# google-research/corenet

Measured on AMD Instinct MI355X. Metric: voxels/sec fwd+bwd @128^3, higher is better.
Workload: dtype bf16x3 (the convolutions of decoder stages 3-6 and the encoder's 3x3 convolutions -- forward of stages 4-5, data gradient of all -- multiply operands split into two bf16 terms: three bf16 MFMAs per product, fp32 accumulation, 16 mantissa bits, ~3e-6 relative per layer; tensors, everything else and t

## Files before the change

corenet_amd/_lib.py:

```python
from __future__ import annotations

import ctypes as C
import os
from typing import Optional

import torch as t

_HERE = os.path.dirname(os.path.abspath(__file__))
TOOLS_LIB_PATH = os.path.join(os.path.dirname(_HERE), "tools", "_build", "libcorenet_hip_tools.so")
PROBE_LIB_PATH = os.path.join(os.path.dirname(_HERE), "tools", "_build", "libcrn_probe.so")
LIB_PATH = os.environ.get("CORENET_HIP_LIB", TOOLS_LIB_PATH if os.environ.get("CRN_TOOLS_LIB") == "1" else
                          os.path.join(_HERE, "lib", "libcorenet_hip.so"))

c_i32p = C.POINTER(C.c_int32)
c_f32p = C.c_void_p
vp = C.c_void_p
i64 = C.c_int64
i32 = C.c_int
f32 = C.c_float
sz = C.c_size_t


class CrnTapBoxes(C.Structure):
  _fields_ = [("n_groups", C.c_int32), ("c_groups", C.c_int32), ("n_box", (C.c_int8 * 6) * 8),
# ... 19 lines not shown
  pass


_SIGS = {
    "crn_conv_fwd": [C.POINTER(CrnView), C.POINTER(CrnInTransform), vp, i32, vp, i32,
                     C.POINTER(CrnView), i32, i32, i32, i32, i32, i32, i32, i32, vp, vp],
    "crn_conv_fwd_bf3": [C.POINTER(CrnView), C.POINTER(CrnInTransform), vp, i32, vp, i32,
                         C.POINTER(CrnView), i32, i32, i32, i32, i32, i32, i32, vp, vp],
    "crn_conv_fwd_bf3_slabs": [C.POINTER(CrnView), C.POINTER(CrnInTransform), vp, i32, vp, i32,
                               C.POINTER(CrnView), i32, i32, i32, i32, i32, i32, i32, vp, vp],
    "crn_conv_fwd_bf3_slabs_bnbwd": [C.POINTER(CrnView), C.POINTER(CrnInTransform), vp, i32, vp, i32,
                                     C.POINTER(CrnView), i32, i32, i32, i32, i32, i32, i32, vp, C.POINTER(CrnBnBwdFuse), vp],
    "crn_conv_fwd_bf3_slabs_stats": [C.POINTER(CrnView), C.POINTER(CrnInTransform), vp, i32, vp, i32,
                                     C.POINTER(CrnView), i32, i32, i32, i32, i32, i32, i32, vp, i32, vp, sz, C.POINTER(C.c_int), vp],
    "crn_batch_renorm_bwd_apply": [vp, i64, vp, i64, i32, i32, i64, i32, vp, vp, vp, vp, vp, i64, vp, vp, i32, vp, i32,
                                   vp, sz, i32, vp],
    "crn_conv_wgrad_bf3": [C.POINTER(CrnView), C.POINTER(CrnInTransform), C.POINTER(CrnView), vp, i32,
                           i32, i32, i32, i32, i32, i32, i32, vp],
    "crn_conv_wgrad_bf3_boxes": [C.POINTER(CrnView), C.POINTER(CrnInTransform), C.POINTER(CrnView), vp, i32,
                                 i32, i32, i32, i32, i32, i32, i32, vp, vp],
    "crn_conv_wgrad": [C.POINTER(CrnView), C.POINTER(CrnInTransform), C.POINTER(CrnView), vp, i32,
                       i32, i32, i32, i32, i32, i32, i32, vp, vp],
    "crn_bf3_operands": [vp, vp, i32, i64, vp, vp],
    "crn_bf3_gather_image": [vp, vp, i32, vp, vp],
    "crn_convt_s2k7_fwd_bf3": [vp, i64, i32, i32, i32, i32, C.POINTER(CrnInTransform), vp, vp, vp, i64, i64, i32, vp],
    "crn_convt_s2k7_dgrad_bf3": [vp, i64, i64, i32, i32, i32, i32, i32, vp, vp, i64, i32, vp],
    "crn_convt_s2k7_c2_fwd_bf3": [vp, i64, i32, i32, i32, i32, C.POINTER(CrnInTransform), vp, vp, vp, i64, i64, i32, vp],
    "crn_convt_s2k7_c2_dgrad_bf3": [vp, i64, i64, i32, i32, i32, i32, i32, vp, vp, i64, i32, vp],
    "crn_convt_s2k7_wgrad_bf3": [vp, i64, i32, i32, i32, i32, C.POINTER(CrnInTransform), vp, i64, i64, i32, vp, i32, i32, vp, vp],
    "crn_convt_s2k7_ximage": [vp, i64, i32, i32, i32, i32, C.POINTER(CrnInTransform), vp, sz, vp],
    "crn_splitk_defer": [i32],
    "crn_splitk_reserve": [i64, vp],
    "crn_splitk_release": [vp],
    "crn_set_deterministic": [i32],
    "crn_roctx_push": [C.c_char_p],
    "crn_roctx_pop": [],
    "crn_comm_unique_id": [vp],
    "crn_comm_init": [vp, i32, i32, C.POINTER(vp)],
    "crn_comm_destroy": [vp],
    "crn_comm_info": [vp, C.POINTER(i32), C.POINTER(i32), C.POINTER(i32)],
    "crn_allreduce_f32": [vp, vp, i64, vp],
    "crn_broadcast_f32": [vp, vp, i64, i32, vp],
    "crn_conv_wgrad_1x1_bf3": [C.POINTER(CrnView), C.POINTER(CrnInTransform), C.POINTER(CrnView), vp, i32, i32, vp],
    "crn_conv_wgrad_2d_bf3": [C.POINTER(CrnView), C.POINTER(CrnInTransform), C.POINTER(CrnView), vp, i32, i32, i32, i32,
                              i32, i32, vp],
    "crn_conv2d_bf3": [C.POINTER(CrnView), C.POINTER(CrnInTransform), vp, i32, vp, i32, C.POINTER(CrnView),
# ... 198 lines not shown
```

corenet_amd/backend.py:

```python
from __future__ import annotations

import ctypes as C
from typing import Optional

import torch as t

from corenet_amd import _lib
from corenet_amd._lib import CrnInTransform, CrnView, ptr
from corenet_amd.views import View, space_to_depth_view, view_of

_DTYPE_CODE = {t.float32: 0, t.uint8: 1, t.int32: 2, t.float64: 3, t.int64: 4, t.int16: 5, t.int8: 6}


def _cview(v: View) -> CrnView:
  base = v.storage.data_ptr() + 4 * (v.offset - v.storage.storage_offset())
  c = v.__dict__.get("_crn")
  if c is None or c[0] != base:
    c = (base, CrnView(base, v.B, v.C, v.D, v.H, v.W, v.sB, v.sC, ptr(v.chan_off), v.sD, v.sH, v.sW))
    object.__setattr__(v, "_crn", c)
  return c[1]


class Transform:
  __slots__ = ("scale", "shift", "pre_relu", "post_relu")
# ... 87 lines not shown
    self.lib.crn_batch_renorm_bwd_apply(ptr(x), sB_x, ptr(g), Cn * S, B, Cn, S, int(pre_relu), ptr(gamma),
                                        ptr(scale), ptr(shift), ptr(saved), ptr(dx), sB_dx, ptr(dgamma), ptr(dbeta),
                                        0, ptr(dsum), int(ndsum), ptr(ws), n, f.nparts, _lib.stream())
    return True

  def splitk_defer(self, on: bool = True):
    self.lib.crn_splitk_defer(int(on))

  def set_deterministic(self, on: bool = True):
    self.lib.crn_set_deterministic(int(on))
    self._deterministic = bool(on)

  def splitk_reserve(self, stream: t.cuda.Stream, floats: int = 0):
    self.lib.crn_splitk_reserve(int(floats), stream.cuda_stream)

  def splitk_release(self, stream: t.cuda.Stream):
    self.lib.crn_splitk_release(stream.cuda_stream)
    for k in [k for k in self._ws if k[0] == "bn@%x" % stream.cuda_stream]:
      del self._ws[k]

  def bf3_operands(self, packed: t.Tensor, table, out: t.Tensor):
    desc, blocks = table
    self.lib.crn_bf3_operands(ptr(packed), ptr(desc), desc.shape[0], blocks, ptr(out), _lib.stream())

  def bf3_gather_image(self, src: t.Tensor, table: t.Tensor, out: t.Tensor, host_table=None):
    self.lib.crn_bf3_gather_image(ptr(src), ptr(table), table.shape[0], ptr(out), _lib.stream())

  def convt_par_fwd(self, x: t.Tensor, tr: Optional[Transform], wimg: t.Tensor, bias: Optional[t.Tensor], y: t.Tensor, cout: int,
                    host_table=None, resident: bool = False):
    B, cin, D, H, W = x.shape
    assert cin == 16 and x[0].is_contiguous() and y[0].is_contiguous() and tuple(y.shape[2:]) == (2 * D, 2 * H, 2 * W)
    fn = self.lib.crn_convt_s2k7_c2_fwd_bf3 if resident else self.lib.crn_convt_s2k7_fwd_bf3
    fn(ptr(x), x.stride(0), B, D, H, W, _ctr(tr), ptr(wimg), ptr(bias), ptr(y), y.stride(0), y.stride(1), cout, _lib.stream())

  def convt_par_dgrad(self, dy: t.Tensor, cout: int, wimg: t.Tensor, dx: t.Tensor, accumulate: bool = False, host_table=None,
                      resident: bool = False):
    B, cin, D, H, W = dx.shape
    assert cin == 16 and dx[0].is_contiguous() and dy[0].is_contiguous() and tuple(dy.shape[2:]) == (2 * D, 2 * H, 2 * W)
    fn = self.lib.crn_convt_s2k7_c2_dgrad_bf3 if resident else self.lib.crn_convt_s2k7_dgrad_bf3
    fn(ptr(dy), dy.stride(0), dy.stride(1), cout, B, D, H, W, ptr(wimg), ptr(dx), dx.stride(0), int(accumulate), _lib.stream())

  def conv2d_bf3(self, x: View, tr: Optional[Transform], wop: t.Tensor, npad: int, bias: Optional[t.Tensor],
                 bias_sB: int, y: View, window, pad_lo, accumulate: bool = False):
    assert window[0] == 1 and pad_lo[0] == 0
    self.lib.crn_conv2d_bf3(C.byref(_cview(x)), _ctr(tr), ptr(wop), npad, ptr(bias), bias_sB, C.byref(_cview(y)),
                            window[1], window[2], pad_lo[1], pad_lo[2], int(accumulate), _lib.stream())
# ... 310 lines not shown
```

corenet_amd/csrc/conv_e2d.hip:

```cpp
#include "conv_kernels.h"
#include "bf3_common.h"
#include <algorithm>
#include <cstdlib>

namespace {
using namespace crnk;

struct E2dGeom {
  crnView x, y;
  crnInTransform tr;
  const void* wop;
  const float* bias;
  int bias_sB;
  int ntn;
  int nblk;
  int ph, pw;
  int tilesH, tilesW;
  int nchunks, chunks_per_split;
  int tab;
  int mode;
  int dbg;
  long long* stamps;
};

// ... 30 lines not shown
    dst[0] = h;
    dst[1] = l;
    return;
  }
  const int ntn = Npad >> 4;
  const long long entries = (long long)(Cin >> 5) * T * ntn * 64;
  const long long e = ((long long)blockIdx.x - d[5]) * 256 + threadIdx.x;
  if (e >= entries) return;
  const int lane = (int)(e & 63);
  const long long rest = e >> 6;
  const int ntile = (int)(rest % ntn);
  const int kg = (int)(rest / ntn);
  const int cbg = kg / T, t = kg - cbg * T;
  const int kk = lane >> 4, i16 = lane & 15;
  const float* src = packed + d[0] + ((long long)(cbg * 32 + kk * 8) * T + t) * Npad + ntile * 16 + i16;
  float v[8];
#pragma unroll
  for (int j = 0; j < 8; ++j) v[j] = src[(long long)j * T * Npad];
  bf16x8 h, l;
  split8(v, h, l);
  bf16x8* dst = reinterpret_cast<bf16x8*>(out + (d[1] + e) * 32);
  dst[0] = h;
  dst[1] = l;
}

constexpr unsigned kOOB = 0x80000000u;

template <int N>
__device__ __forceinline__ void wait_vm(f32x4& a, f32x4& b) {
  asm volatile("s_waitcnt vmcnt(%2)" : "+v"(a), "+v"(b) : "n"(N));
}

template <int T, int CB, int TW>
__global__ __launch_bounds__(256, 2) void conv_e2d_kernel(E2dGeom g) {
  constexpr int KW = T == 9 ? 3 : 1;
  constexpr int TH = 64 / TW, PH = TH + KW - 1, PW = TW + KW - 1, NPOS = PH * PW;
  constexpr int NPA = T == 9 ? 128 : 64;
  constexpr int KS = CB * T;
  constexpr int NPL = T == 9 ? 16 : 8;
  constexpr int PS = NPA + 4;
  constexpr int PLANE = CB * 4 * PS;
  static_assert(T == 9 ? CB == 1 : CB == 4, "thread -> patch element mapping");
  extern __shared__ __attribute__((aligned(16))) char smem[];
  float* tscale = reinterpret_cast<float*>(smem);
  float* tshift = tscale + g.tab;
  bf16x8* Abuf = reinterpret_cast<bf16x8*>(smem + (size_t)g.tab * 8);
// ... 514 lines not shown
    const int mt = tile >> 1, nt = tile & 1, qt = mt / 3, zw = mt - 3 * qt;
    const int n = n0 + 16 * nt + i16;
#pragma unroll
    for (int r = 0; r < 4; ++r) {
      const int q = q0 + 16 * qt + 4 * kk + r;
      if (q < 3 * g.C && n < g.N) atomicAdd(g.dw + (long long)(3 * q + zw) * g.Npad + n, v[r]);
    }
  }
}

bool dense_2d(const crnView& v) {
  return v.chan_off == nullptr && v.sW == 1 && v.sH == v.W && (v.D == 1 || v.sD == v.H * v.W) && (v.sC & 3) == 0 &&
         (v.sB & 3) == 0 && (((uintptr_t)v.base) & 15) == 0;
}

}

extern "C" int crn_bf3_operands(const float* packed, const int64_t* desc, int nlayers, int64_t total_blocks, void* out,
                                crnStream stream) {
  CRN_ENTRY(stream);
  if (!packed || !desc || !out || nlayers < 1 || total_blocks < 1 || total_blocks > 0x7fffffff) return CRN_EINVAL;
  hipLaunchKernelGGL(bf3_operands_kernel, dim3((unsigned)total_blocks), dim3(256), 0, (hipStream_t)stream, packed,
                     reinterpret_cast<const long long*>(desc), nlayers, reinterpret_cast<char*>(out));
  CRN_CHECK_LAUNCH();
  return CRN_OK;
}

namespace {
long long* g_stamps = nullptr;
template <int T, int CB, int TW>
int launch_e2d(const E2dGeom& g, dim3 grid, size_t lds, hipStream_t st) {
  return crn_launch(conv_e2d_kernel<T, CB, TW>, grid, dim3(256), lds, st, g);
}
}

extern "C" int crn_conv2d_bf3(const crnView* x, const crnInTransform* tr, const void* wop, int Npad, const float* bias,
                              int bias_sB, const crnView* y, int kh, int kw, int ph, int pw, int accumulate,
                              crnStream stream) {
  if (!x || !y || !wop || x->B != y->B || x->B < 1) return CRN_EINVAL;
  if (!dense_2d(*x) || !dense_2d(*y)) return CRN_EINVAL;
  if ((x->C & 31) || (y->C & 63) || Npad != y->C) return CRN_EINVAL;
  if (x->D != y->D || x->H != y->H || x->W != y->W) return CRN_EINVAL;
  const bool k3 = kh == 3 && kw == 3, k1 = kh == 1 && kw == 1;
  if (!k3 && !k1) return CRN_EINVAL;
  if (k1 && (ph || pw)) return CRN_EINVAL;
  const int64_t S = (int64_t)x->D * x->H * x->W;
// ... 135 lines not shown
```

corenet_amd/model/conv_geometry.py:

```python
from __future__ import annotations

import dataclasses
from typing import Tuple

import numpy as np


def pad16(n: int) -> int:
  return (n + 15) // 16 * 16


@dataclasses.dataclass
class Geom:
  window: Tuple[int, int, int]
  pad_lo: Tuple[int, int, int]
  index: np.ndarray
  cin: int
  nout: int
  npad: int
  n_boxes: Tuple = ()
  c_boxes: Tuple = ()

  @property
  def taps(self) -> int:
    return self.window[0] * self.window[1] * self.window[2]


def _k3(shape_tail):
  k = tuple(shape_tail)
  return (1,) * (3 - len(k)) + k


def conv_fwd(wshape, padding) -> Geom:
  N, Cc = wshape[:2]
  k = _k3(wshape[2:])
  T = k[0] * k[1] * k[2]
  npad = pad16(N)
  idx = np.full((Cc, T, npad), -1, np.int64)
  n = np.arange(N)[None, None, :]
  c = np.arange(Cc)[:, None, None]
  tt = np.arange(T)[None, :, None]
  idx[:, :, :N] = (n * Cc + c) * T + tt
  p = _k3((padding,) * (len(wshape) - 2)) if np.isscalar(padding) else _k3(padding)
  if len(wshape) == 4:
    p = (0,) + tuple(p[1:])
  return Geom(k, tuple(p), idx.reshape(-1).astype(np.int32), Cc, N, npad)


def conv_dgrad(wshape, padding) -> Geom:
  N, Cc = wshape[:2]
  k = _k3(wshape[2:])
  T = k[0] * k[1] * k[2]
  npad = pad16(Cc)
  idx = np.full((N, T, npad), -1, np.int64)
  n = np.arange(N)[:, None, None]
  c = np.arange(Cc)[None, None, :]
  tt = np.arange(T)[None, :, None]
  idx[:, :, :Cc] = (n * Cc + c) * T + (T - 1 - tt)
  p = _k3((padding,) * (len(wshape) - 2)) if np.isscalar(padding) else _k3(padding)
  if len(wshape) == 4:
    p = (0,) + tuple(p[1:])
  pad = tuple(kk - 1 - pp for kk, pp in zip(k, p))
  return Geom(k, pad, idx.reshape(-1).astype(np.int32), N, Cc, npad)


def _convt_ranges(ks: int, p: int):
  dmin = -((ks - 1 - p) // 2)
  dmax = (1 + p) // 2
  emin = (0 - p) // 2
  emax = (ks - 1 - p) // 2
  return dmin, dmax, emin, emax


def _parity_boxes(valid_r_w: np.ndarray):
  rng = []
  for r in range(2):
    pos = np.nonzero(valid_r_w[r])[0]
    assert len(pos) > 0 and (np.diff(pos) == 1).all()
    rng.append((int(pos[0]), int(pos[-1]) + 1))
  return tuple(rng[rd] + rng[rh] + rng[rw] for rd in range(2) for rh in range(2) for rw in range(2))


def convt_fwd(wshape, padding: int) -> Geom:
  Cc, N, ks = wshape[0], wshape[1], wshape[2]
  dmin, dmax, _, _ = _convt_ranges(ks, padding)
  nw = dmax - dmin + 1
  npad = pad16(N * 8)
  wq = np.arange(nw)
  r = np.arange(2)
  kk = -2 * (wq[:, None] + dmin) + r[None, :] + padding
  valid1 = (kk >= 0) & (kk < ks)
  c = np.arange(Cc).reshape(Cc, 1, 1, 1, 1, 1, 1, 1)
  n = np.arange(N).reshape(1, 1, 1, 1, N, 1, 1, 1)
  kd = kk.reshape(1, nw, 1, 1, 1, 2, 1, 1); vd = valid1.reshape(1, nw, 1, 1, 1, 2, 1, 1)
  kh = kk.reshape(1, 1, nw, 1, 1, 1, 2, 1); vh = valid1.reshape(1, 1, nw, 1, 1, 1, 2, 1)
  kw = kk.reshape(1, 1, 1, nw, 1, 1, 1, 2); vw = valid1.reshape(1, 1, 1, nw, 1, 1, 1, 2)
  flat = (((c * N + n) * ks + kd) * ks + kh) * ks + kw
  flat = np.where(vd & vh & vw, flat, -1)
  flat = flat.transpose(0, 1, 2, 3, 5, 6, 7, 4)
  idx = np.full((Cc, nw ** 3, npad), -1, np.int64)
  idx[:, :, :N * 8] = flat.reshape(Cc, nw ** 3, N * 8)
  return Geom((nw,) * 3, (-dmin,) * 3, idx.reshape(-1).astype(np.int32), Cc, N * 8, npad,
              n_boxes=_parity_boxes(valid1.T))


def convt_dgrad(wshape, padding: int) -> Geom:
  Cc, N, ks = wshape[0], wshape[1], wshape[2]
  _, _, emin, emax = _convt_ranges(ks, padding)
  nw = emax - emin + 1
  npad = pad16(Cc)
  wq = np.arange(nw)
  r = np.arange(2)
  kk = 2 * (wq[None, :] + emin) + r[:, None] + padding
  valid1 = (kk >= 0) & (kk < ks)
  n = np.arange(N).reshape(N, 1, 1, 1, 1, 1, 1, 1)
  c = np.arange(Cc).reshape(1, 1, 1, 1, 1, 1, 1, Cc)
  kd = kk.reshape(1, 2, 1, 1, nw, 1, 1, 1); vd = valid1.reshape(1, 2, 1, 1, nw, 1, 1, 1)
  kh = kk.reshape(1, 1, 2, 1, 1, nw, 1, 1); vh = valid1.reshape(1, 1, 2, 1, 1, nw, 1, 1)
  kw = kk.reshape(1, 1, 1, 2, 1, 1, nw, 1); vw = valid1.reshape(1, 1, 1, 2, 1, 1, nw, 1)
  flat = (((c * N + n) * ks + kd) * ks + kh) * ks + kw
  flat = np.where(vd & vh & vw, flat, -1)
  flat = flat.transpose(1, 2, 3, 0, 4, 5, 6, 7)
  idx = np.full((N * 8, nw ** 3, npad), -1, np.int64)
  idx[:, :, :Cc] = flat.reshape(N * 8, nw ** 3, Cc)
  return Geom((nw,) * 3, (-emin,) * 3, idx.reshape(-1).astype(np.int32), N * 8, Cc, npad,
              c_boxes=_parity_boxes(valid1))


def stem_fwd(wshape=(64, 3, 7, 7), padding: int = 3) -> Geom:
  N, Cc, ks, _ = wshape
  emin, emax = (0 - padding) // 2, (ks - 1 - padding) // 2
  nw = emax - emin + 1
  npad = pad16(N)
  wq = np.arange(nw); r = np.arange(2)
  kk = 2 * (wq[None, :] + emin) + r[:, None] + padding
  valid1 = (kk >= 0) & (kk < ks)
  c = np.arange(Cc).reshape(Cc, 1, 1, 1, 1, 1)
  n = np.arange(N).reshape(1, 1, 1, 1, 1, N)
  kh = kk.reshape(1, 2, 1, nw, 1, 1); vh = valid1.reshape(1, 2, 1, nw, 1, 1)
  kw = kk.reshape(1, 1, 2, 1, nw, 1); vw = valid1.reshape(1, 1, 2, 1, nw, 1)
  flat = ((n * Cc + c) * ks + kh) * ks + kw
  flat = np.where(vh & vw, flat, -1)
  idx = np.full((Cc * 4, nw * nw, npad), -1, np.int64)
  idx[:, :, :N] = flat.reshape(Cc * 4, nw * nw, N)
  return Geom((1, nw, nw), (0, -emin, -emin), idx.reshape(-1).astype(np.int32), Cc * 4, N, npad)


def convt_1to4_fwd(wshape) -> Geom:
  Cc, N = wshape[0], wshape[1]
# ... 129 lines not shown
  return (g.window in ((1, 1, 1), (1, 3, 3)) and g.cin % 32 == 0 and g.nout % 64 == 0 and g.npad == g.nout
          and not g.n_boxes and not g.c_boxes)


def operand_entries(g: Geom) -> int:
  return (g.cin // 32) * g.taps * (g.npad // 16) * 64


def slab_entries(g: Geom) -> int:
  khw = g.window[1] * g.window[2]
  return ((g.cin + 7) // 8) * g.window[0] * ((khw + 3) // 4 * 4) * g.npad


def operand_table(layers):
  rows, blocks = [], 0
  for layer in layers:
    src, dst, g = layer[:3]
    slab = len(layer) > 3 and layer[3]
    rows.append((src, dst, g.cin, g.taps, g.npad, blocks, g.window[1] * g.window[2] if slab else 0))
    blocks += ((slab_entries(g) if slab else operand_entries(g)) + 255) // 256
  return np.asarray(rows, dtype=np.int64).reshape(-1, 7), blocks


def _ct_table(rows_of_step):
  tab, off16 = [], 0
  for rows, entry in rows_of_step:
    hi0, lo0 = off16, off16 + rows * 128
    for zi in range(rows):
      for kk in range(4):
        for col in range(32):
          e = (zi * 4 + kk) * 32 + col
          tab.append(list(entry(zi, kk, col)) + [hi0 + e, lo0 + e])
    off16 += rows * 256
  return np.asarray(tab, np.int32), off16 * 16 + 4096


def convt_par_fwd_table(wshape, wofs: int = 0):
  Cc, N, ks = wshape[0], wshape[1], wshape[2]
  assert Cc == 16 and ks == 7 and N <= 16
  steps = []
  for pp in range(4):
    rd, rh = pp >> 1, pp & 1
    for ch in range(2):
      for zd in range(3 + rd):
        def entry(zh, kk, col, rd=rd, rh=rh, ch=ch, zd=zd):
          rw, n = col >> 4, col & 15
# ... 65 lines not shown
```

corenet_amd/model/engine.py:

```python
from __future__ import annotations

import dataclasses
import os
from typing import Dict, List, Optional, Tuple

import numpy as np
import torch as t

from corenet_amd import _lib
from corenet_amd import views as V
from corenet_amd.backend import Transform
from corenet_amd.model import conv_geometry as G

IMAGE_HW = (256, 256)


def check_image_hw(hw):
  H, W = int(hw[0]), int(hw[1])
  if H < 32 or W < 32 or H % 4 or W % 4 or H * W > 4096 * 4096:
    raise ValueError(f"corenet_amd.CoreNet: image batch of {H}x{W} pixels; this engine takes H and W that are multiples of 4 and >= 32 "
                     f"(256x256 in every shipped config)")
  return H, W
BN_EPS = 1e-3
BN_MOMENTUM = 0.01

ENC_STAGES = (("stage2", "abc", (64, 64, 256), 1), ("stage3", "abcd", (128, 128, 512), 2),
# ... 326 lines not shown
        add(name, G.convt_1to4_fwd(shape), G.convt_1to4_dgrad(shape), repeat=64)
      elif ".t1." in name:
        p = 1 if shape[2] == 3 else 3
        add(name, G.convt_fwd(shape, p), G.convt_dgrad(shape, p), repeat=8)
      else:
        p = shape[-1] // 2
        add(name, G.conv_fwd(shape, p), G.conv_dgrad(shape, p))
    idx_parts, sizes = [], []
    for name, fwd, dgrad, repeat, nref in reg:
      wo, bo = s.offset(name + "weight"), s.offset(name + "bias")
      def shift(ix, o):
        return np.where(ix >= 0, ix.astype(np.int64) + o, -1)
      parts = [shift(fwd.index, wo), shift(G.bias_index(nref, repeat, fwd.npad, parity_major=(repeat == 8)), bo)]
      if dgrad is not None:
        alias = (len(dgrad.index) == int(np.prod(s.off[name + "weight"][1]))
                 and np.array_equal(dgrad.index, np.arange(len(dgrad.index))))
        parts.append(np.zeros(0, np.int64) if alias else shift(dgrad.index, wo))
      idx_parts.append(parts)
    flat_len = sum(len(p) for parts in idx_parts for p in parts)
    assert max(int(p.max()) for parts in idx_parts for p in parts if len(p)) < 2 ** 31
    self.packed = t.zeros(flat_len, dtype=self.dtype, device=self.device)
    gsize = sum(len(parts[0]) for parts in idx_parts)
    self.gpacked = t.zeros(gsize, dtype=self.dtype, device=self.device)
    pack_parts, pack_is_bwd, pack_names, unpack_parts = [], [], [], []
    po, go = 0, 0
    for (name, fwd, dgrad, repeat, nref), parts in zip(reg, idx_parts):
      pack_parts.append((po, parts[0], fwd.npad, 0)); po += len(parts[0]); pack_is_bwd.append(False); pack_names.append(name)
      pack_parts.append((po, parts[1], len(parts[1]), 0)); po += len(parts[1]); pack_is_bwd.append(False); pack_names.append(name)
      if dgrad is not None and len(parts[2]):
        pack_parts.append((po, parts[2], dgrad.npad, dgrad.taps if dgrad.taps > 1 else 0)); po += len(parts[2])
        pack_is_bwd.append(True); pack_names.append(name)
      unpack_parts.append((go, parts[0], fwd.npad, 0)); go += len(parts[0])
    dev = self._tiles_dev
    self.pack_tiles = dev([pp for pp, bwd in zip(pack_parts, pack_is_bwd) if not bwd])
    sel = lambda pred: [pp for pp, bwd, nm in zip(pack_parts, pack_is_bwd, pack_names) if not bwd and pred(nm)]
    early = lambda nm: nm.startswith("encoder.stage1") or nm.startswith("encoder.stage2")
    self.pack_tiles_enc = dev(sel(lambda nm: nm.startswith("encoder.")))
    self.pack_tiles_enc_early = dev(sel(early))
    self.pack_tiles_enc_late = dev(sel(lambda nm: nm.startswith("encoder.") and not early(nm)))
    self.pack_tiles_dec = dev(sel(lambda nm: not nm.startswith("encoder.")))
    self.pack_tiles_bwd = dev([pp for pp, bwd in zip(pack_parts, pack_is_bwd) if bwd])
    self.unpack_tiles = dev(unpack_parts)
    los = [min(o for k, (o, _) in s.off.items() if s.kind[k] == "param" and k.startswith(lb))
           for lb in GRAD_BUCKET_LABELS[:-1]] + [0]
    self.grad_buckets: List[Tuple[str, int, int]] = []
    self._bucket_tiles = []
    hi = s.params.numel()
    for lb, lo in zip(GRAD_BUCKET_LABELS, los):
      assert lo < hi
      self.grad_buckets.append((lb, lo, hi))
      sel = [up for (name, *_), up in zip(reg, unpack_parts) if lo <= s.offset(name + "weight") < hi]
      self._bucket_tiles.append(sel)
      hi = lo
    self._bucket_dev = None
    po, go = 0, 0
    for (name, fwd, dgrad, repeat, nref), parts in zip(reg, idx_parts):
      nwf, nb = len(parts[0]), len(parts[1])
      wf = self.packed[po:po + nwf]; po += nwf
      bias = self.packed[po:po + nb]; po += nb
      wd = None
      if dgrad is not None:
        if len(parts[2]):
          wd = self.packed[po:po + len(parts[2])]; po += len(parts[2])
        else:
          wd = s.view(name + "weight").view(-1)
# ... 5 lines not shown
  def _build_ct_images(self):
    self.ct_tables = {}
    name = "decoder.stage_6.t1."
    if (self.decoder_math != "bf16x3" or self.device.type != "cuda"
        or name not in self.convs or not hasattr(self.be, "convt_par_fwd")):
      return
    shape = tuple(self.store.off[name + "weight"][1])
    if shape[0] != 16 or shape[1] > 16 or tuple(shape[2:]) != (7, 7, 7) or tuple(self.resolution) != (128, 128, 128):
      return
    if shape[1] == 2:
      kind_, tabs = "res", (G.convt_res_fwd_table, G.convt_res_dgrad_table)
    elif shape[1] >= CT_PAR_MIN:
      kind_, tabs = "par", (G.convt_par_fwd_table, G.convt_par_dgrad_table)
    else:
      return
    self.convs[name].ct_kind = kind_
    wofs = self.store.offset(name + "weight")
    for kind, fn, field in (("dec", tabs[0], "ct_f"), ("bwd", tabs[1], "ct_d")):
      tab, nbytes = fn(shape, wofs)
      img = t.zeros(nbytes, dtype=t.uint8, device=self.device)
      setattr(self.convs[name], field, img)
      self.ct_tables[kind] = (t.as_tensor(tab, device=self.device), img)

  def _build_operands(self, reg, idx_parts):
    self.wop = None
    self.op_tables = {}
    self._build_ct_images()
    if self.decoder_math != "bf16x3":
      return
    groups = {"enc_early": [], "enc_late": [], "dec": [], "bwd": []}
    slices = []
    po, eo = 0, 0
    for (name, fwd, dgrad, repeat, nref), parts in zip(reg, idx_parts):
      src_f = po; po += len(parts[0]) + len(parts[1])
      src_d = po
      if dgrad is not None:
        po += len(parts[2])
      if (name, "fwd") in BF16X3_LAUNCHES:
        groups["dec"].append((src_f, eo, fwd, True))
        slices.append((name, "wop_f", eo, G.slab_entries(fwd))); eo += G.slab_entries(fwd)
        groups["bwd"].append((src_d, eo, dgrad, True))
        slices.append((name, "wop_d", eo, G.slab_entries(dgrad))); eo += G.slab_entries(dgrad)
        self.convs[name].wop_kind = "slab"
        continue
      if not self.encoder_e2d or not name.startswith("encoder.") or name.startswith("encoder.stage1"):
        continue
      self.convs[name].wop_kind = "e2d"
      if fwd.window != (1, 3, 3):
        continue
      if G.operand_eligible(fwd) and name[len("encoder.stage")] in "45":
        groups["enc_early" if name.startswith("encoder.stage2") else "enc_late"].append((src_f, eo, fwd))
        slices.append((name, "wop_f", eo, G.operand_entries(fwd))); eo += G.operand_entries(fwd)
      if dgrad is not None and len(parts[2]) and G.operand_eligible(dgrad):
        groups["bwd"].append((src_d, eo, dgrad))
        slices.append((name, "wop_d", eo, G.operand_entries(dgrad))); eo += G.operand_entries(dgrad)
    if not eo:
      return
    self.wop = t.zeros(eo * 32, dtype=t.uint8, device=self.device)
    for name, field, e0, n in slices:
      setattr(self.convs[name], field, self.wop[e0 * 32:(e0 + n) * 32])
    for k, layers in groups.items():
      if layers:
        desc, blocks = G.operand_table(layers)
        self.op_tables[k] = (t.as_tensor(desc, device=self.device), blocks)

  def _operands(self, *groups):
    for k in groups:
      if k in self.op_tables:
        self.be.bf3_operands(self.packed, self.op_tables[k], self.wop)
      if k in self.ct_tables:
        self.be.bf3_gather_image(self.store.params, *self.ct_tables[k])

  def _tiles_dev(self, parts):
    mats, rest = G.mat_index(parts)
    tl = G.tile_index(rest)
    return (t.as_tensor(tl[0], device=self.device), t.as_tensor(tl[1].view(np.int64), device=self.device),
            t.as_tensor(tl[2] if tl[2].size else np.zeros(1, np.int32), device=self.device),
            t.as_tensor(mats, device=self.device))

  def bucket_unpack_tiles(self, i: int):
    if self._bucket_dev is None:
      self._bucket_dev = [self._tiles_dev(sel) for sel in self._bucket_tiles]
    return self._bucket_dev[i]

  @property
  def weights_dirty(self) -> bool:
    return self._weights_dirty

  @weights_dirty.setter
  def weights_dirty(self, v: bool):
    self._weights_dirty = v
    if v:
      self.dgrad_dirty = True

  def pack_weights(self, part: str = "all"):
    tiles = {"all": self.pack_tiles, "enc": self.pack_tiles_enc, "dec": self.pack_tiles_dec,
             "enc_early": self.pack_tiles_enc_early, "enc_late": self.pack_tiles_enc_late}[part]
    self.be.copy_tiles(self.store.params, self.packed, tiles)
    self._operands(*{"all": ("enc_early", "enc_late", "dec"), "enc": ("enc_early", "enc_late"), "dec": ("dec",),
                     "enc_early": ("enc_early",), "enc_late": ("enc_late",)}[part])
    if part in ("all", "dec"):
      self._weights_dirty = False

  def pack_dgrad_weights(self):
    self.be.copy_tiles(self.store.params, self.packed, self.pack_tiles_bwd)
    self._operands("bwd")
    self.dgrad_dirty = False

  def plan(self, batch: int, hw=IMAGE_HW) -> "Plan":
    hw = (int(hw[0]), int(hw[1]))
    key = batch if hw == IMAGE_HW else (batch, hw[0], hw[1])
    p = self.plans.get(key)
    if p is None:
      p = Plan(self, batch, hw)
      self.plans[key] = p
    return p

  def adam_step(self, lr: float, eps: float, betas=(0.9, 0.999), grad_scale: float = 1.0):
    if self.adam_m is None:
      self.adam_m = t.zeros_like(self.store.params)
      self.adam_v = t.zeros_like(self.store.params)
    self.adam_t += 1
    self.be.adam_step(self.store.params, self.store.grads, self.adam_m, self.adam_v,
                      self.store.params.numel(), lr, betas[0], betas[1], eps, grad_scale, self.adam_t)
    self.weights_dirty = True

  def adam_step_graphable(self, lr: float, eps: float, betas=(0.9, 0.999), grad_scale: float = 1.0, launch: bool = True):
    if self.adam_m is None:
# ... 52 lines not shown
    self.gy1 = f(B, 64, *self.stem_hw); self.gy1b = f(B, 64, *self.stem_hw)
    self.p1 = f(B, 64, *self.pool_hw)
    self.p1_arg = t.zeros(B, 64, *self.pool_hw, dtype=t.int32, device=dev)
    self.blocks = []
    cin, (hi, wi) = 64, self.pool_hw
    stage_hw = {}
    for name, blocks, filt, stride in ENC_STAGES:
      for bl in blocks:
        st = stride if bl == "a" else 1
        ho, wo = (hi + st - 1) // st, (wi + st - 1) // st
        z = lambda c: f(B, c, ho, wo)
        s2 = st == 2
        blk = EncBlock(prefix=f"encoder.{name}.{bl}.", stage=name, cin=cin, f=filt, stride=st, h=ho, w=wo, down=(bl == "a"),
                       final=(bl == blocks[-1]), ya=z(filt[0]), yb=z(filt[1]), yc=z(filt[2]), ys=z(filt[2]) if bl == "a" else None,
                       out=z(filt[2]), gpre=z(filt[2]), gyc=z(filt[2]), gab=z(filt[1]), gyb=z(filt[1]), gaa=z(filt[0]), gya=z(filt[0]),
                       gys=z(filt[2]) if bl == "a" else None, gin=f(B, cin, hi, wi) if bl == "a" else None,
                       xs=z(cin) if s2 else None, gxs=z(cin) if s2 else None)
        if s2 and self.blocks:
          self.blocks[-1].xs_next = blk
        self.blocks.append(blk)
        cin, hi, wi = filt[2], ho, wo
      stage_hw[name] = (hi, wi)
    self.stage_hw = stage_hw
    self.feat = {"stage2": f(B, 256 + 3, *stage_hw["stage2"]), "stage3": f(B, 512 + 3, *stage_hw["stage3"]),
                 "stage4": f(B, 1024 + 3, *stage_hw["stage4"]), "stage5": f(B, 2048 + 3, *stage_hw["stage5"])}
    self.gfeat = {k: t.zeros_like(v) for k, v in self.feat.items()}
    self.avg = f(B, 2048); self.gavg = f(B, 2048)
    L = eng.latent
    self.z0 = f(B, L + 3); self.gz0 = f(B, L + 3); self.gv0 = f(B, L + 3)
    C = eng.num_classes
    sk = eng.skip_ch
    self.dec = {}
    for k, (ci, cm, co, r) in {2: (256, 256, 128, 4), 3: (128 + sk[2], 128, 64, 8), 4: (64 + sk[3], 64, 32, 16),
                               5: (32 + sk[4], 32, 16, 32), 6: (16 + sk[5], 16, C, 64)}.items():
      self.dec[k] = DecStage(ci, cm, co, r, u=f(B, ci, r, r, r), gu=f(B, ci, r, r, r), w=f(B, cm, r, r, r), gw=f(B, cm, r, r, r),
                             gv1=f(B, ci, r, r, r), gv2=f(B, cm, r, r, r))
    self.logits = f(B, C, 128, 128, 128)
    self.glogits = f(B, C, 128, 128, 128)
    self.skip_src = {2: "stage5", 3: "stage4", 4: "stage3", 5: "stage2"}
    self.skip_hw = {k: stage_hw[self.skip_src[k]] for k in self.skip_src}
    self.smap = {k: f(B, self.skip_hw[k][0], self.skip_hw[k][1], sk[k]) for k in sk}
    self.ray_idx = ({k: t.zeros(B, (2 * self.dec[k].r) ** 3, dtype=t.int16, device=dev) for k in sk}
                    if hasattr(self.be, "ray_sample_fwd_idx") and max(h * w for h, w in self.skip_hw.values()) < 65535 else None)
    gs_n = {k: B * sk[k] * self.skip_hw[k][0] * self.skip_hw[k][1] for k in sk}
    self.gsmap_slab = f(sum(gs_n.values()))
    self.gsmap, o = {}, 0
# ... 626 lines not shown
```

include/corenet_hip.h:

```cpp
#ifndef CORENET_HIP_H_
#define CORENET_HIP_H_

#include <stddef.h>
#include <stdint.h>

#ifdef __cplusplus
extern "C" {
#endif

#define CRN_OK 0
#define CRN_EINVAL (-1)
#define CRN_ENOMEM (-2)
#define CRN_ENOCONV (-3)

typedef void* crnStream;

typedef struct {
  float* base;
  int32_t B, C, D, H, W;
  int64_t sB, sC;
  const int32_t* chan_off;
  int32_t sD, sH, sW;
} crnView;

// ... 44 lines not shown
                                 const float* bias, int bias_sB, const crnView* y,
                                 int kd, int kh, int kw, int pd, int ph, int pw,
                                 int accumulate, const crnTapBoxes* boxes , int pre_relu,
                                 double* ws, size_t ws_bytes, int* nparts, crnStream stream);

int crn_splitk_defer(int on);
int crn_splitk_reserve(int64_t floats, crnStream stream);
int crn_splitk_release(crnStream stream);

int crn_conv_wgrad(const crnView* x, const crnInTransform* tr, const crnView* dy,
                   float* dw, int Npad, int kd, int kh, int kw, int pd, int ph, int pw,
                   int zero_first, const crnTapBoxes* boxes ,
                   crnStream stream);

int crn_conv_wgrad_bf3(const crnView* x, const crnInTransform* tr, const crnView* dy,
                       float* dw, int Npad, int kd, int kh, int kw, int pd, int ph, int pw,
                       int zero_first, crnStream stream);
int crn_conv_wgrad_bf3_boxes(const crnView* x, const crnInTransform* tr, const crnView* dy, float* dw, int Npad,
                             int kd, int kh, int kw, int pd, int ph, int pw, int zero_first,
                             const crnTapBoxes* boxes , crnStream stream);

int crn_bf3_operands(const float* packed, const int64_t* desc, int nlayers, int64_t total_blocks, void* out,
                     crnStream stream);
int crn_conv2d_bf3(const crnView* x, const crnInTransform* tr, const void* wop, int Npad, const float* bias,
                   int bias_sB, const crnView* y, int kh, int kw, int ph, int pw, int accumulate, crnStream stream);

int crn_conv_wgrad_1x1_bf3(const crnView* x, const crnInTransform* tr, const crnView* dy, float* dw, int Npad,
                           int zero_first, crnStream stream);
int crn_conv_wgrad_2d_bf3(const crnView* x, const crnInTransform* tr, const crnView* dy, float* dw, int Npad,
                          int kh, int kw, int ph, int pw, int zero_first, crnStream stream);

int crn_copy_tiles_f32(const float* src, float* dst, const int32_t* desc ,
                       const uint64_t* mask , const int32_t* explicit_idx, int64_t ntiles,
                       int reverse, crnStream s);
int crn_copy_mats_f32(const float* src, float* dst, const int32_t* desc , int64_t nblocks,
                      int reverse, crnStream s);
int crn_gather_f32(const float* src, const int32_t* idx, float* dst, int64_t n, crnStream s);
int crn_scatter_f32(const float* src, const int32_t* idx, float* dst, int64_t n,
                    int accumulate, crnStream s);
int crn_bias_grad(const float* dy, int B, int C, int64_t S, int64_t sB, float* db,
                  int accumulate, double* workspace ,
                  size_t workspace_bytes, crnStream s);

int crn_batch_renorm_stats(const float* x, int B, int C, int64_t S, int64_t sB, int pre_relu,
                           const float* gamma, const float* beta,
                           float* running_mean, float* running_var,
// ... 230 lines not shown
```

Before: 1.209 billion.

## Build bf16x3 weight operands directly from parameters, skipping fp32 packed images

Adds a kernel that reads weights straight from the parameter store with stride-based index arithmetic. It transposes them through LDS and writes the split bf16 hi/lo operands. Layers converted this way are dropped from the fp32 tile-copy pack tables, so the per-step copy into the packed image is skipped for them. A fallback restores the full packs when an encoder block shape needs fp32 images, at the cost of a more complex gather kernel with integer magic-number division.

```diff
diff --git a/corenet_amd/_lib.py b/corenet_amd/_lib.py
--- a/corenet_amd/_lib.py
+++ b/corenet_amd/_lib.py
@@ -65,6 +65,7 @@
     "crn_conv_wgrad": [C.POINTER(CrnView), C.POINTER(CrnInTransform), C.POINTER(CrnView), vp, i32,
                        i32, i32, i32, i32, i32, i32, i32, vp, vp],
     "crn_bf3_operands": [vp, vp, i32, i64, vp, vp],
+    "crn_bf3_operands_from_params": [vp, vp, i32, i64, vp, vp],
     "crn_bf3_gather_image": [vp, vp, i32, vp, vp],
     "crn_convt_s2k7_fwd_bf3": [vp, i64, i32, i32, i32, i32, C.POINTER(CrnInTransform), vp, vp, vp, i64, i64, i32, vp],
     "crn_convt_s2k7_dgrad_bf3": [vp, i64, i64, i32, i32, i32, i32, i32, vp, vp, i64, i32, vp],
diff --git a/corenet_amd/backend.py b/corenet_amd/backend.py
--- a/corenet_amd/backend.py
+++ b/corenet_amd/backend.py
@@ -133,6 +133,10 @@
   def bf3_operands(self, packed: t.Tensor, table, out: t.Tensor):
     desc, blocks = table
     self.lib.crn_bf3_operands(ptr(packed), ptr(desc), desc.shape[0], blocks, ptr(out), _lib.stream())
+
+  def bf3_operands_from_params(self, params: t.Tensor, table, out: t.Tensor):
+    desc, blocks = table
+    self.lib.crn_bf3_operands_from_params(ptr(params), ptr(desc), desc.shape[0], blocks, ptr(out), _lib.stream())
 
   def bf3_gather_image(self, src: t.Tensor, table: t.Tensor, out: t.Tensor, host_table=None):
     self.lib.crn_bf3_gather_image(ptr(src), ptr(table), table.shape[0], ptr(out), _lib.stream())
diff --git a/corenet_amd/csrc/conv_e2d.hip b/corenet_amd/csrc/conv_e2d.hip
--- a/corenet_amd/csrc/conv_e2d.hip
+++ b/corenet_amd/csrc/conv_e2d.hip
@@ -76,6 +76,98 @@
   bf16x8* dst = reinterpret_cast<bf16x8*>(out + (d[1] + e) * 32);
   dst[0] = h;
   dst[1] = l;
+}
+
+constexpr int kSrcFields = 32;
+constexpr int kSrcLds = 8192;
+__device__ __forceinline__ int src_div(int x, unsigned magic) { return magic ? (int)__umulhi((unsigned)x, magic) : x; }
+
+__global__ __launch_bounds__(256) void bf3_operands_from_params_kernel(const float* __restrict__ params,
+                                                                       const long long* __restrict__ desc, int nlayers,
+                                                                       char* __restrict__ out) {
+  __shared__ float tile[kSrcLds];
+  int lo = 0, hi = nlayers - 1;
+  while (lo < hi) {
+    const int mid = (lo + hi + 1) >> 1;
+    if (desc[mid * kSrcFields + 5] <= (long long)blockIdx.x) lo = mid; else hi = mid - 1;
+  }
+  const long long* d = desc + lo * kSrcFields;
+  const long long base = d[0], sr = d[7], sq = d[8];
+  const int Cin = (int)d[2], T = (int)d[3], Npad = (int)d[4], KHW = (int)d[6];
+  const int RN = (int)d[9], QN = (int)d[10], nreal = (int)d[11], par = (int)d[12], a = (int)d[13];
+  const int k0d = (int)d[14], k0h = (int)d[15], k0w = (int)d[16];
+  const unsigned ksd = (unsigned)d[17], ksh = (unsigned)d[18], ksw = (unsigned)d[19];
+  const int nww = (int)d[20], QB = (int)d[21], ord = (int)d[22], nqb = (int)d[27];
+  const unsigned mTB = (unsigned)d[23], mMT = (unsigned)d[24], mW = (unsigned)d[25], mP = (unsigned)d[26];
+  const bool blocks = KHW == 0;
+  const int taps = blocks ? T : KHW;
+  const int TB = blocks ? T : (KHW + 3) & ~3;
+  const int kd = blocks ? 1 : T / KHW;
+  const int RB = blocks ? 32 : 8;
+  const int QBP = QB + 1;
+  const int b = (int)((long long)blockIdx.x - d[5]);
+  const int rest = b / nqb, qb = b - rest * nqb;
+  const int rb = blocks ? rest : rest / kd, zd = blocks ? 0 : rest - rb * kd;
+  const int r0 = rb * RB, q0 = qb * QB;
+  const int MT = (ord ? QB : RB) * TB, nel = RB * TB * QB;
+  constexpr int U = 8;
+  for (int e0 = threadIdx.x; e0 < nel; e0 += 256 * U) {
+    int l[U];
+    float val[U];
+#pragma unroll
+    for (int u = 0; u < U; ++u) {
+      const int e = e0 + u * 256;
+      l[u] = -1;
+      val[u] = 0.f;
+      if (e >= nel) continue;
+      const int o = src_div(e, mMT), rem = e - o * MT, m = src_div(rem, mTB), tp = rem - m * TB;
+      const int j = ord ? o : m, i = ord ? m : o;
+      l[u] = (j * TB + tp) * QBP + i;
+      const int row = r0 + j, col = q0 + i;
+      if (row >= Cin || col >= nreal || tp >= taps) continue;
+      int rr = row, qq = col, p = 0;
+      if (par == 1) { p = src_div(row, mP); rr = row - p * RN; }
+      else if (par == 2) { p = src_div(col, mP); qq = col - p * QN; }
+      const int wh = src_div(tp, mW), ww = tp - wh * nww;
+      const int kz = a * zd + (p >> 2) + k0d, ky = a * wh + ((p >> 1) & 1) + k0h, kx = a * ww + (p & 1) + k0w;
+      if ((unsigned)kz < ksd && (unsigned)ky < ksh && (unsigned)kx < ksw)
+        val[u] = params[base + rr * sr + qq * sq + (long long)((kz * (int)ksh + ky) * (int)ksw + kx)];
+    }
+#pragma unroll
+    for (int u = 0; u < U; ++u)
+      if (l[u] >= 0) tile[l[u]] = val[u];
+  }
+  __syncthreads();
+  if (blocks) {
+    const int ntn = Npad >> 4;
+    for (int x = threadIdx.x; x < TB * 64; x += 256) {
+      const int t = x >> 6, lane = x & 63, kk = lane >> 4, i16 = lane & 15;
+      float v[8];
+#pragma unroll
+      for (int j = 0; j < 8; ++j) v[j] = tile[((kk * 8 + j) * TB + t) * QBP + i16];
+      bf16x8 h, l;
+      split8(v, h, l);
+      const long long e = (((long long)rb * T + t) * ntn + qb) * 64 + lane;
+      bf16x8* dst = reinterpret_cast<bf16x8*>(out + (d[1] + e) * 32);
+      dst[0] = h;
+      dst[1] = l;
+    }
+    return;
+  }
+  const int qsh = QB == 32 ? 5 : 4, ncol = min(QB, Npad - q0);
+  for (int x = threadIdx.x; x < TB * QB; x += 256) {
+    const int tp = x >> qsh, i = x & (QB - 1);
+    if (i >= ncol) continue;
+    float v[8];
+#pragma unroll
+    for (int j = 0; j < 8; ++j) v[j] = tile[(j * TB + tp) * QBP + i];
+    bf16x8 h, l;
+    split8(v, h, l);
+    const long long e = ((long long)rest * TB + tp) * Npad + q0 + i;
+    bf16x8* dst = reinterpret_cast<bf16x8*>(out + (d[1] + e) * 32);
+    dst[0] = h;
+    dst[1] = l;
+  }
 }
 
 constexpr unsigned kOOB = 0x80000000u;
@@ -636,6 +728,16 @@
   if (!packed || !desc || !out || nlayers < 1 || total_blocks < 1 || total_blocks > 0x7fffffff) return CRN_EINVAL;
   hipLaunchKernelGGL(bf3_operands_kernel, dim3((unsigned)total_blocks), dim3(256), 0, (hipStream_t)stream, packed,
                      reinterpret_cast<const long long*>(desc), nlayers, reinterpret_cast<char*>(out));
+  CRN_CHECK_LAUNCH();
+  return CRN_OK;
+}
+
+extern "C" int crn_bf3_operands_from_params(const float* params, const int64_t* desc, int nlayers, int64_t total_blocks,
+                                            void* out, crnStream stream) {
+  CRN_ENTRY(stream);
+  if (!params || !desc || !out || nlayers < 1 || total_blocks < 1 || total_blocks > 0x7fffffff) return CRN_EINVAL;
+  hipLaunchKernelGGL(bf3_operands_from_params_kernel, dim3((unsigned)total_blocks), dim3(256), 0, (hipStream_t)stream,
+                     params, reinterpret_cast<const long long*>(desc), nlayers, reinterpret_cast<char*>(out));
   CRN_CHECK_LAUNCH();
   return CRN_OK;
 }
diff --git a/corenet_amd/model/conv_geometry.py b/corenet_amd/model/conv_geometry.py
--- a/corenet_amd/model/conv_geometry.py
+++ b/corenet_amd/model/conv_geometry.py
@@ -20,6 +20,7 @@
   npad: int
   n_boxes: Tuple = ()
   c_boxes: Tuple = ()
+  src: Tuple = ()
 
   @property
   def taps(self) -> int:
@@ -44,7 +45,8 @@
   p = _k3((padding,) * (len(wshape) - 2)) if np.isscalar(padding) else _k3(padding)
   if len(wshape) == 4:
     p = (0,) + tuple(p[1:])
-  return Geom(k, tuple(p), idx.reshape(-1).astype(np.int32), Cc, N, npad)
+  return Geom(k, tuple(p), idx.reshape(-1).astype(np.int32), Cc, N, npad,
+              src=(T, Cc * T, Cc, N, 0, 1, (0, 0, 0), k))
 
 
 def conv_dgrad(wshape, padding) -> Geom:
@@ -61,7 +63,8 @@
   if len(wshape) == 4:
     p = (0,) + tuple(p[1:])
   pad = tuple(kk - 1 - pp for kk, pp in zip(k, p))
-  return Geom(k, pad, idx.reshape(-1).astype(np.int32), N, Cc, npad)
+  return Geom(k, pad, idx.reshape(-1).astype(np.int32), N, Cc, npad,
+              src=(Cc * T, T, N, Cc, 0, -1, tuple(kk - 1 for kk in k), k))
 
 
 def _convt_ranges(ks: int, p: int):
@@ -101,7 +104,8 @@
   idx = np.full((Cc, nw ** 3, npad), -1, np.int64)
   idx[:, :, :N * 8] = flat.reshape(Cc, nw ** 3, N * 8)
   return Geom((nw,) * 3, (-dmin,) * 3, idx.reshape(-1).astype(np.int32), Cc, N * 8, npad,
-              n_boxes=_parity_boxes(valid1.T))
+              n_boxes=_parity_boxes(valid1.T),
+              src=(N * ks ** 3, ks ** 3, Cc, N, 2, -2, (padding - 2 * dmin,) * 3, (ks,) * 3))
 
 
 def convt_dgrad(wshape, padding: int) -> Geom:
@@ -124,7 +128,8 @@
   idx = np.full((N * 8, nw ** 3, npad), -1, np.int64)
   idx[:, :, :Cc] = flat.reshape(N * 8, nw ** 3, Cc)
   return Geom((nw,) * 3, (-emin,) * 3, idx.reshape(-1).astype(np.int32), N * 8, Cc, npad,
-              c_boxes=_parity_boxes(valid1))
+              c_boxes=_parity_boxes(valid1),
+              src=(ks ** 3, N * ks ** 3, N, Cc, 1, 2, (padding + 2 * emin,) * 3, (ks,) * 3))
 
 
 def stem_fwd(wshape=(64, 3, 7, 7), padding: int = 3) -> Geom:
@@ -300,6 +305,124 @@
   return np.asarray(rows, dtype=np.int64).reshape(-1, 7), blocks
 
 
+SRC_FIELDS = 32
+SRC_LDS = 8192
+
+
+def _magic(q: int) -> int:
+  return 0 if q == 1 else ((1 << 32) + q - 1) // q
+
+
+def source_index(g: Geom) -> np.ndarray:
+  sr, sq, RN, QN, par, a, k0, ks = g.src
+  row = np.arange(g.cin).reshape(-1, 1, 1, 1, 1)
+  col = np.arange(g.npad).reshape(1, 1, 1, 1, -1)
+  w = [np.arange(g.window[i]).reshape([-1 if j == i else 1 for j in range(3)] ) for i in range(3)]
+  w = [x.reshape((1,) + x.shape + (1,)) for x in w]
+  p = row // RN if par == 1 else col // QN if par == 2 else 0 * row
+  rr = row % RN if par == 1 else row
+  qq = col % QN if par == 2 else col
+  k = [a * w[i] + ((p >> (2 - i)) & 1) + k0[i] for i in range(3)]
+  ok = (col < g.nout) & (p < 8)
+  for i in range(3):
+    ok = ok & (k[i] >= 0) & (k[i] < ks[i])
+  flat = rr * sr + qq * sq + (k[0] * ks[1] + k[1]) * ks[2] + k[2]
+  return np.where(ok, flat, -1).reshape(-1).astype(np.int64)
+
+
+def direct_operand_table(layers):
+  rows, blocks = [], 0
+  for layer in layers:
+    wofs, dst, g = layer[:3]
+    slab = len(layer) > 3 and layer[3]
+    assert g.src, "no stride description of this layout"
+    sr, sq, RN, QN, par, a, k0, ks = g.src
+    khw = g.window[1] * g.window[2]
+    if slab:
+      TB, RB = (khw + 3) // 4 * 4, 8
+      QB = 32 if g.npad % 32 == 0 and RB * TB * 33 <= SRC_LDS else 16
+      nrb = (g.cin + 7) // 8 * g.window[0]
+    else:
+      assert g.window[0] == 1 and g.cin % 32 == 0
+      TB, RB, QB = g.taps, 32, 16
+      nrb = g.cin // 32
+    assert RB * TB * (QB + 1) <= SRC_LDS and max(g.cin, g.npad, RB * TB * QB) < 2 ** 16, (g.window, g.cin, g.npad)
+    nqb = (g.npad + QB - 1) // QB
+    order = 0 if sr < sq else 1
+    mid = (QB if order else RB) * TB
+    row = [wofs, dst, g.cin, g.taps, g.npad, blocks, khw if slab else 0, sr, sq, RN, QN, g.nout, par, a, *k0, *ks,
+           g.window[2], QB, order, _magic(TB), _magic(mid), _magic(g.window[2]), _magic(RN if par == 1 else QN), nqb]
+    rows.append(row + [0] * (SRC_FIELDS - len(row)))
+    blocks += nrb * nqb
+  return np.asarray(rows, dtype=np.int64).reshape(-1, SRC_FIELDS), blocks
+
+
+def operand_entry_positions(g: Geom, slab: bool) -> np.ndarray:
+  T, Npad = g.taps, g.npad
+  j = np.arange(8)[None, :]
+  if slab:
+    khw, kd = g.window[1] * g.window[2], g.window[0]
+    TP = (khw + 3) // 4 * 4
+    e = np.arange(slab_entries(g))[:, None]
+    n, r = e % Npad, e // Npad
+    tp, r = r % TP, r // TP
+    zd, chunk = r % kd, r // kd
+    c = chunk * 8 + j
+    return np.where((c < g.cin) & (tp < khw), (c * T + zd * khw + tp) * Npad + n, -1)
+  ntn = Npad // 16
+  e = np.arange(operand_entries(g))[:, None]
+  lane, rest = e & 63, e >> 6
+  ntile, kg = rest % ntn, rest // ntn
+  cbg, tt = kg // T, kg % T
+  return ((cbg * 32 + (lane >> 4) * 8 + j) * T + tt) * Npad + ntile * 16 + (lane & 15)
+
+
+def direct_entry_sources(row) -> np.ndarray:
+  d = [int(x) for x in row]
+  base, Cin, T, Npad, KHW, sr, sq, RN, QN, nreal, par, a = d[0], d[2], d[3], d[4], d[6], d[7], d[8], d[9], d[10], d[11], d[12], d[13]
+  k0, ks, nww, QB, nqb = d[14:17], d[17:20], d[20], d[21], d[27]
+  mW, mP = d[25], d[26]
+  div = lambda x, m: (x * m) >> 32 if m else x
+  blocks_ = KHW == 0
+  taps = T if blocks_ else KHW
+  TB = T if blocks_ else (KHW + 3) // 4 * 4
+  kd = 1 if blocks_ else T // KHW
+  RB = 32 if blocks_ else 8
+  nrb = (Cin // 32) if blocks_ else (Cin + 7) // 8 * kd
+  n_entries = (Cin // 32) * T * (Npad // 16) * 64 if blocks_ else (Cin + 7) // 8 * kd * TB * Npad
+  out = np.full((n_entries, 8), -2, np.int64)
+  b = np.arange(nrb * nqb).reshape(-1, 1, 1)
+  rest, qb = b // nqb, b % nqb
+  rb, zd = (rest, 0 * rest) if blocks_ else (rest // kd, rest % kd)
+  jj = np.arange(8).reshape(1, 1, 8)
+  if blocks_:
+    x = np.arange(TB * 64).reshape(1, -1, 1)
+    tp, lane = x >> 6, x & 63
+    j, i = (lane >> 4) * 8 + jj, lane & 15
+    e = ((rb * T + tp) * (Npad // 16) + qb) * 64 + lane
+    keep = np.ones_like(e, bool)
+  else:
+    x = np.arange(TB * QB).reshape(1, -1, 1)
+    tp, i = x // QB, x % QB
+    j = jj
+    e = (rest * TB + tp) * Npad + qb * QB + i
+    keep = (qb * QB + i < Npad) & (e >= 0)
+  rowi, col = rb * RB + j, qb * QB + i
+  p = div(rowi, mP) if par == 1 else div(col, mP) if par == 2 else 0 * rowi
+  rr = rowi - p * RN if par == 1 else rowi
+  qq = col - p * QN if par == 2 else col
+  wh = div(tp, mW); ww = tp - wh * nww
+  kz, ky, kx = a * zd + (p >> 2) + k0[0], a * wh + ((p >> 1) & 1) + k0[1], a * ww + (p & 1) + k0[2]
+  ok = (rowi < Cin) & (col < nreal) & (tp < taps) & (kz >= 0) & (kz < ks[0]) & (ky >= 0) & (ky < ks[1]) & (kx >= 0) & (kx < ks[2])
+  srcv = np.where(ok, base + rr * sr + qq * sq + (kz * ks[1] + ky) * ks[2] + kx, -1)
+  e, keep, srcv = np.broadcast_arrays(e, keep, srcv)
+  ee = e[..., 0][keep[..., 0]]
+  if len(np.unique(ee)) != len(ee) or len(ee) != n_entries or ee.min() != 0 or ee.max() != n_entries - 1:
+    raise ValueError("the workgroups do not cover the layer's entries exactly once")
+  out[ee] = srcv[keep[..., 0]]
+  return out
+
+
 def _ct_table(rows_of_step):
   tab, off16 = [], 0
   for rows, entry in rows_of_step:
diff --git a/corenet_amd/model/engine.py b/corenet_amd/model/engine.py
--- a/corenet_amd/model/engine.py
+++ b/corenet_amd/model/engine.py
@@ -2,6 +2,7 @@
 
 import dataclasses
 import os
+import types
 from typing import Dict, List, Optional, Tuple
 
 import numpy as np
@@ -374,25 +375,16 @@
     self.packed = t.zeros(flat_len, dtype=self.dtype, device=self.device)
     gsize = sum(len(parts[0]) for parts in idx_parts)
     self.gpacked = t.zeros(gsize, dtype=self.dtype, device=self.device)
-    pack_parts, pack_is_bwd, pack_names, unpack_parts = [], [], [], []
+    pack_parts, unpack_parts = [], []
     po, go = 0, 0
     for (name, fwd, dgrad, repeat, nref), parts in zip(reg, idx_parts):
-      pack_parts.append((po, parts[0], fwd.npad, 0)); po += len(parts[0]); pack_is_bwd.append(False); pack_names.append(name)
-      pack_parts.append((po, parts[1], len(parts[1]), 0)); po += len(parts[1]); pack_is_bwd.append(False); pack_names.append(name)
+      pack_parts.append(((po, parts[0], fwd.npad, 0), name, "w")); po += len(parts[0])
+      pack_parts.append(((po, parts[1], len(parts[1]), 0), name, "b")); po += len(parts[1])
       if dgrad is not None and len(parts[2]):
-        pack_parts.append((po, parts[2], dgrad.npad, dgrad.taps if dgrad.taps > 1 else 0)); po += len(parts[2])
-        pack_is_bwd.append(True); pack_names.append(name)
+        pack_parts.append(((po, parts[2], dgrad.npad, dgrad.taps if dgrad.taps > 1 else 0), name, "d")); po += len(parts[2])
       unpack_parts.append((go, parts[0], fwd.npad, 0)); go += len(parts[0])
-    dev = self._tiles_dev
-    self.pack_tiles = dev([pp for pp, bwd in zip(pack_parts, pack_is_bwd) if not bwd])
-    sel = lambda pred: [pp for pp, bwd, nm in zip(pack_parts, pack_is_bwd, pack_names) if not bwd and pred(nm)]
-    early = lambda nm: nm.startswith("encoder.stage1") or nm.startswith("encoder.stage2")
-    self.pack_tiles_enc = dev(sel(lambda nm: nm.startswith("encoder.")))
-    self.pack_tiles_enc_early = dev(sel(early))
-    self.pack_tiles_enc_late = dev(sel(lambda nm: nm.startswith("encoder.") and not early(nm)))
-    self.pack_tiles_dec = dev(sel(lambda nm: not nm.startswith("encoder.")))
-    self.pack_tiles_bwd = dev([pp for pp, bwd in zip(pack_parts, pack_is_bwd) if bwd])
-    self.unpack_tiles = dev(unpack_parts)
+    self._pack_parts = pack_parts
+    self.unpack_tiles = self._tiles_dev(unpack_parts)
     los = [min(o for k, (o, _) in s.off.items() if s.kind[k] == "param" and k.startswith(lb))
            for lb in GRAD_BUCKET_LABELS[:-1]] + [0]
     self.grad_buckets: List[Tuple[str, int, int]] = []
@@ -444,24 +436,40 @@
       setattr(self.convs[name], field, img)
       self.ct_tables[kind] = (t.as_tensor(tab, device=self.device), img)
 
+  def _pack_tables(self, skip=frozenset()):
+    sel = lambda pred: self._tiles_dev([pp for pp, nm, kind in self._pack_parts if (nm, kind) not in skip and pred(nm, kind)])
+    early = lambda nm: nm.startswith("encoder.stage1") or nm.startswith("encoder.stage2")
+    return {"all": sel(lambda nm, kind: kind != "d"),
+            "enc": sel(lambda nm, kind: kind != "d" and nm.startswith("encoder.")),
+            "enc_early": sel(lambda nm, kind: kind != "d" and early(nm)),
+            "enc_late": sel(lambda nm, kind: kind != "d" and nm.startswith("encoder.") and not early(nm)),
+            "dec": sel(lambda nm, kind: kind != "d" and not nm.startswith("encoder.")),
+            "bwd": sel(lambda nm, kind: kind == "d")}
+
   def _build_operands(self, reg, idx_parts):
     self.wop = None
     self.op_tables = {}
+    self.direct_tables = {}
     self._build_ct_images()
+    self.fp32_images = True
+    self._packs_full = None
     if self.decoder_math != "bf16x3":
+      self._packs = self._pack_tables()
       return
     groups = {"enc_early": [], "enc_late": [], "dec": [], "bwd": []}
+    direct = {k: [] for k in groups}
     slices = []
     po, eo = 0, 0
     for (name, fwd, dgrad, repeat, nref), parts in zip(reg, idx_parts):
+      wo = self.store.offset(name + "weight")
       src_f = po; po += len(parts[0]) + len(parts[1])
       src_d = po
       if dgrad is not None:
         po += len(parts[2])
       if (name, "fwd") in BF16X3_LAUNCHES:
-        groups["dec"].append((src_f, eo, fwd, True))
+        groups["dec"].append((src_f, eo, fwd, True)); direct["dec"].append((wo, eo, fwd, True))
         slices.append((name, "wop_f", eo, G.slab_entries(fwd))); eo += G.slab_entries(fwd)
-        groups["bwd"].append((src_d, eo, dgrad, True))
+        groups["bwd"].append((src_d, eo, dgrad, True)); direct["bwd"].append((wo, eo, dgrad, True))
         slices.append((name, "wop_d", eo, G.slab_entries(dgrad))); eo += G.slab_entries(dgrad)
         self.convs[name].wop_kind = "slab"
         continue
@@ -471,12 +479,14 @@
       if fwd.window != (1, 3, 3):
         continue
       if G.operand_eligible(fwd) and name[len("encoder.stage")] in "45":
-        groups["enc_early" if name.startswith("encoder.stage2") else "enc_late"].append((src_f, eo, fwd))
+        k = "enc_early" if name.startswith("encoder.stage2") else "enc_late"
+        groups[k].append((src_f, eo, fwd)); direct[k].append((wo, eo, fwd))
         slices.append((name, "wop_f", eo, G.operand_entries(fwd))); eo += G.operand_entries(fwd)
       if dgrad is not None and len(parts[2]) and G.operand_eligible(dgrad):
-        groups["bwd"].append((src_d, eo, dgrad))
+        groups["bwd"].append((src_d, eo, dgrad)); direct["bwd"].append((wo, eo, dgrad))
         slices.append((name, "wop_d", eo, G.operand_entries(dgrad))); eo += G.operand_entries(dgrad)
     if not eo:
+      self._packs = self._pack_tables()
       return
     self.wop = t.zeros(eo * 32, dtype=t.uint8, device=self.device)
     for name, field, e0, n in slices:
@@ -485,11 +495,32 @@
       if layers:
         desc, blocks = G.operand_table(layers)
         self.op_tables[k] = (t.as_tensor(desc, device=self.device), blocks)
+    if not hasattr(self.be, "bf3_operands_from_params"):
+      self._packs = self._pack_tables()
+      return
+    for k, layers in direct.items():
+      if layers:
+        desc, blocks = G.direct_operand_table(layers)
+        self.direct_tables[k] = (t.as_tensor(desc, device=self.device), blocks)
+    self.fp32_images = False
+    self._packs = self._pack_tables(frozenset((name, "w" if field == "wop_f" else "d") for name, field, _, _ in slices))
+
+  def need_fp32_images(self):
+    if self.fp32_images:
+      return
+    if self._packs_full is None:
+      self._packs_full = self._pack_tables()
+    self._packs = self._packs_full
+    self.fp32_images = True
+    self.weights_dirty = True
 
   def _operands(self, *groups):
     for k in groups:
-      if k in self.op_tables:
-        self.be.bf3_operands(self.packed, self.op_tables[k], self.wop)
+      if self.fp32_images:
+        if k in self.op_tables:
+          self.be.bf3_operands(self.packed, self.op_tables[k], self.wop)
+      elif k in self.direct_tables:
+        self.be.bf3_operands_from_params(self.store.params, self.direct_tables[k], self.wop)
       if k in self.ct_tables:
         self.be.bf3_gather_image(self.store.params, *self.ct_tables[k])
 
@@ -516,16 +547,14 @@
       self.dgrad_dirty = True
 
   def pack_weights(self, part: str = "all"):
-    tiles = {"all": self.pack_tiles, "enc": self.pack_tiles_enc, "dec": self.pack_tiles_dec,
-             "enc_early": self.pack_tiles_enc_early, "enc_late": self.pack_tiles_enc_late}[part]
-    self.be.copy_tiles(self.store.params, self.packed, tiles)
+    self.be.copy_tiles(self.store.params, self.packed, self._packs[part])
     self._operands(*{"all": ("enc_early", "enc_late", "dec"), "enc": ("enc_early", "enc_late"), "dec": ("dec",),
                      "enc_early": ("enc_early",), "enc_late": ("enc_late",)}[part])
     if part in ("all", "dec"):
       self._weights_dirty = False
 
   def pack_dgrad_weights(self):
-    self.be.copy_tiles(self.store.params, self.packed, self.pack_tiles_bwd)
+    self.be.copy_tiles(self.store.params, self.packed, self._packs["bwd"])
     self._operands("bwd")
     self.dgrad_dirty = False
 
@@ -624,6 +653,9 @@
         cin, hi, wi = filt[2], ho, wo
       stage_hw[name] = (hi, wi)
     self.stage_hw = stage_hw
+    extent = lambda blk: types.SimpleNamespace(D=1, H=blk.h, W=blk.w)
+    if eng.wop is not None and not all(self._e2d_shape_ok(extent(blk), (1, 3, 3)) for blk in self.blocks):
+      eng.need_fp32_images()
     self.feat = {"stage2": f(B, 256 + 3, *stage_hw["stage2"]), "stage3": f(B, 512 + 3, *stage_hw["stage3"]),
                  "stage4": f(B, 1024 + 3, *stage_hw["stage4"]), "stage5": f(B, 2048 + 3, *stage_hw["stage5"])}
     self.gfeat = {k: t.zeros_like(v) for k, v in self.feat.items()}
diff --git a/include/corenet_hip.h b/include/corenet_hip.h
--- a/include/corenet_hip.h
+++ b/include/corenet_hip.h
@@ -90,6 +90,8 @@
 
 int crn_bf3_operands(const float* packed, const int64_t* desc, int nlayers, int64_t total_blocks, void* out,
                      crnStream stream);
+int crn_bf3_operands_from_params(const float* params, const int64_t* desc, int nlayers, int64_t total_blocks, void* out,
+                                 crnStream stream);
 int crn_conv2d_bf3(const crnView* x, const crnInTransform* tr, const void* wop, int Npad, const float* bias,
                    int bias_sB, const crnView* y, int kh, int kw, int ph, int pw, int accumulate, crnStream stream);
 
```

Result: no change. 1.208 billion (-0.2%).
